# iwbn/flow-supervisor

Hardware: AMD Instinct MI355X
Metric: image-pairs/s fwd+bwd, 12 GRU iters, 436x1024 (higher is better)
Workload: dtype f32 (bf16x3 products); 1 GPU; RAFT full, 440x1024 (Sintel 436x1024 padded), 12 GRU iters, 4 pairs/GPU, train step = fwd + sequence loss + bwd + RCCL all-reduce + clip + AdamW; global_batch=4, parallelism=dp1, launch=hipGraph replay of the whole step

## Files before the change

flow_supervisor_amd/_lib.py:

```python
import ctypes
import functools
import os
from ctypes import POINTER, Structure, c_double, c_float, c_int, c_int64, c_void_p

import torch

_HERE = os.path.dirname(os.path.abspath(__file__))
LIB_PATH = os.environ.get("FSRAFT_LIB_PATH") or os.path.join(_HERE, "libfsraft.so")
_lib = None

c_float_p = c_void_p


class ConvDesc(Structure):
    _fields_ = [
        ("src", c_void_p * 3), ("srcC", c_int * 3), ("srcld", c_int * 3), ("nsrc", c_int),
        ("wpk", c_void_p), ("bias", c_void_p), ("wpk_split", c_void_p),
        ("B", c_int), ("H", c_int), ("W", c_int), ("KH", c_int), ("KW", c_int), ("N", c_int),
        ("dst", c_void_p * 3), ("dst_bs", c_int64 * 3), ("dst_ps", c_int64 * 3), ("dst_cs", c_int64 * 3),
        ("dst_n0", c_int * 3), ("dst_acc", c_int * 3), ("ndst", c_int),
        ("relu", c_int), ("alpha", c_float),
        ("epi", c_int),
        ("h", c_void_p), ("ldh", c_int), ("z", c_void_p), ("ldz", c_int),
        ("aux1", c_void_p), ("ld1", c_int), ("aux2", c_void_p), ("ld2", c_int), ("hid", c_int),
# ... 83 lines not shown
    "fsraft_inorm_relu_fwd": [c_void_p, c_void_p, c_void_p, c_int64, c_int, c_float, c_int, _S],
    "fsraft_inorm_relu_bwd": [c_void_p, c_void_p, c_void_p, c_void_p, c_int64, c_int, c_int, _S],
    "fsraft_affine_relu_fwd": [c_void_p, c_void_p, c_void_p, c_void_p, c_int64, c_int, c_int, c_int, _S],
    "fsraft_affine_relu_bwd": [c_void_p, c_void_p, c_void_p, c_void_p, c_void_p, c_void_p, c_void_p, c_int64, c_int, c_int, c_int, _S],
    "fsraft_sequence_loss": [_PP, _PP, POINTER(c_float), c_int, c_int, c_void_p, c_void_p, c_float, c_float, c_int, c_int, c_int, c_void_p, _S],
    "fsraft_corr_pool_pyramid": [_PP, c_int, c_int64, c_int, c_int, _S],
    "fsraft_corr_pool_pyramid_same": [_PP, c_int, c_int64, c_int, c_int, _S],
    "fsraft_corr_lookup_fwd_same": [_PP, c_int, c_void_p, c_int64, c_int64, c_int64, c_void_p, c_int, c_int, c_int, c_int, c_int, _S],
    "fsraft_corr_unpool_same_bwd": [_PP, c_int, c_int64, c_int, c_int, _S],
    "fsraft_corr_lookup_bwd_same": [_PP, c_int, c_void_p, c_int64, c_int64, c_int64, c_void_p, c_int, c_int, c_int, c_int, c_int, _S],
    "fsraft_corr_lookup_dcoords_same": [_PP, c_int, c_void_p, c_int64, c_int64, c_int64, c_void_p, c_int, c_void_p, c_int64, c_int64, c_int64,
                                        c_int, c_int, c_int, c_int, _S],
    "fsraft_set_norm_blocks": [c_int],
    "fsraft_get_tuning": [c_int],
    "fsraft_conv_last_route": [c_int],
    "fsraft_space_to_depth2": [c_void_p, c_void_p, c_int, c_int, c_int, c_int, c_int, _S],
    "fsraft_forward_interpolate": [c_void_p, c_void_p, c_int, c_int, _S],
    "fsraft_flow_metrics_scratch_bytes": [c_int, c_int, c_int],
    "fsraft_flow_metrics": [c_void_p, c_int64, c_int64, c_int64, c_void_p, c_int64, c_int64, c_int64, c_void_p, c_int64, c_int64,
                            c_int, c_int, c_int, c_void_p, c_void_p, c_void_p, c_int64, _S],
    "fsraft_inorm_relu_cl_fwd": [c_void_p, c_void_p, c_void_p, c_void_p, c_void_p, c_void_p, c_int, c_int, c_int, c_float, c_int, c_int, c_int, _S],
    "fsraft_inorm_relu_cl_bwd": [c_void_p, c_void_p, c_void_p, c_void_p, c_void_p, c_void_p, c_void_p, c_void_p, c_int, c_int, c_int,
                                 c_int, c_int, _S],
    "fsraft_affine_relu_cl_fwd": [c_void_p, c_void_p, c_void_p, c_void_p, c_void_p, c_int64, c_int, c_int, c_int, c_int, _S],
    "fsraft_affine_relu_cl_bwd": [c_void_p, c_void_p, c_void_p, c_void_p, c_void_p, c_void_p, c_void_p, c_void_p, c_void_p, c_int, c_int,
                                  c_int, c_int, c_int, _S],
    "fsraft_axpby": [c_void_p, c_void_p, c_float, c_float, c_int64, _S],
    "fsraft_sum_n": [_PP, c_int, c_void_p, c_int64, c_int, _S],
    "fsraft_bn_fold": [c_void_p, c_void_p, c_void_p, c_void_p, c_void_p, c_float, c_int, c_void_p, c_void_p, c_void_p, c_void_p, _S],
    "fsraft_bn_fold_bwd": [c_void_p, c_int, c_int, c_void_p, c_void_p, c_void_p, c_void_p, c_void_p, c_void_p, _S],
# ... 145 lines not shown
```

flow_supervisor_amd/csrc/conv_common.hpp:

```cpp
#pragma once
#include "gemm_core.hpp"
#include "gemm_core_split.hpp"
#include "gemm_rec.hpp"
#include <cstddef>
#include <type_traits>

struct ConvKnobs {
  int conv_tile = 0;
  int wgrad_tile = 0;
  int wgrad_blocks = 512;
  int conv_split = 1;
  int wgrad_split = 2;
  int conv_buf = 1;
  int xcd_swizzle = 0;
  int wgrad_buf = 1;
  int conv_n256 = 0;
  int wgrad_multi = 1;
  int wgrad_blocks_multi = 2048;
  int conv_uniform = 1;
  int conv_w8 = 1;
  int conv_w8_min = 64;
  int wgrad_w8 = 0;
  int wgrad_pack = 1;
  int wgrad_blocks_pack = 1024;
// ... 53 lines not shown
__device__ __forceinline__ const T* uni_ptr(const T* p) {
  const uint64_t u = reinterpret_cast<uint64_t>(p);
  return reinterpret_cast<const T*>((uint64_t)uni((unsigned)(u >> 32)) << 32 | uni((unsigned)u));
}
__device__ __forceinline__ __amdgpu_buffer_rsrc_t make_rsrc(const void* p, unsigned bytes) {
  const uint64_t u = reinterpret_cast<uint64_t>(p);
  const unsigned lo = __builtin_amdgcn_readfirstlane((unsigned)u), hi = __builtin_amdgcn_readfirstlane((unsigned)(u >> 32));
  void* q = reinterpret_cast<void*>((uint64_t)hi << 32 | lo);
  return __builtin_amdgcn_make_buffer_rsrc(q, 0, __builtin_amdgcn_readfirstlane(bytes), FS_RSRC_FLAGS);
}

using SWCfg128 = SplitTnCfg<128, 128, 2, 2, 2>;
using SWCfg128S = SplitTnCfg<128, 128, 2, 2, 1>;
using SWCfg128W8 = SplitTnCfg<128, 128, 2, 4, 1, 512>;
using SWCfgPack = SplitTnCfg<64, 192, 2, 2, 1>;
using Cfg128 = GemmCfg<128, 128, 32, 2, 2, 2, 2>;
using Cfg64 = GemmCfg<128, 64, 32, 4, 1, 2, 2>;
using CfgM64 = GemmCfg<64, 128, 32, 1, 4, 2, 2>;
using Cfg6464 = GemmCfg<64, 64, 32, 2, 2, 2, 2>;
using WCfg6464 = GemmCfg<64, 64, 32, 2, 2, 0, 0>;
using Cfg6464K16 = GemmCfg<64, 64, 16, 2, 2, 2, 2>;
using CfgM64K16 = GemmCfg<64, 128, 16, 1, 4, 2, 2>;

using SCfg128 = SplitCfg<128, 128, 2, 2>;
using SCfgN256 = SplitCfg<64, 256, 1, 4, 2, true>;
using SCfg256W16 = SplitCfg<256, 128, 4, 4, 2, true, 1024>;
using SCfg128W8 = SplitCfg<128, 128, 2, 4, 2, true, 512>;
using SCfg256N64 = SplitCfg<256, 64, 4, 2, 2, true, 512>;
using SCfgM64 = SplitCfg<64, 128, 1, 4, 2, true>;
using Cfg32 = GemmCfg<128, 32, 32, 4, 1, 2, 2>;
// ... 47 lines not shown
```

flow_supervisor_amd/csrc/conv_wgrad.hip:

```cpp
#include "conv_common.hpp"

namespace {

struct WgradArgs {
  const float* dy; int ldy; int Cout;
  Src src[3]; int nsrc;
  float* dwpk; int Ktot;
  int B, H, W, KH, KW;
  int kchunk;
  float* dbias;
  int xcd_xt, xcd_yt, xcd_groups;
};

constexpr int WGRAD_MAX_SEG = 16;
struct WgradArgsM {
  WgradArgs a;
  int nseg, zs;
  const float* dys[WGRAD_MAX_SEG];
  const float* srcs[3][WGRAD_MAX_SEG];
};

template <class Cfg>
struct ShiftedXLoader {
  static constexpr int BN = Cfg::BN, BK = Cfg::BK, LD = Cfg::LDB;
  static constexpr int F4 = BN / 4;
  static constexpr int NF4 = BK * F4 / 256;
// ... 109 lines not shown
    const int ku = __builtin_amdgcn_readfirstlane(kt);
    const unsigned w = __builtin_amdgcn_readfirstlane(mask[ku]);
    const __amdgpu_buffer_rsrc_t rs = make_rsrc(base, 0x7fffffffu);
    const unsigned soff = (unsigned)ku * 32u * ld4;
#pragma unroll
    for (int j = 0; j < NCH; ++j) {
      const unsigned voffj = voff[j] | ((__builtin_amdgcn_ubfe(w, (unsigned)krow[j], 1u) ^ 1u) << 31);
      const u32x4 v = __builtin_amdgcn_raw_buffer_load_b128(rs, voffj, soff, 0);
      const f32x4 f = __builtin_bit_cast(f32x4, v);
      r[4 * j + 0] = f[0]; r[4 * j + 1] = f[1]; r[4 * j + 2] = f[2]; r[4 * j + 3] = f[3];
    }
  }
};


template <class Cfg, bool BUF = false, bool MULTI = false>
__global__ __launch_bounds__(Cfg::NT) void conv_wgrad_split_kernel(const std::conditional_t<MULTI, WgradArgsM, WgradArgs> args) {
  static_assert(Cfg::NT == 256 || BUF, "512-thread workgroups use the buffer-addressed loaders");
  __shared__ __attribute__((aligned(16))) char lds[Cfg::LDS_BYTES];
  __shared__ unsigned pixmask[BUF ? WGRAD_MASK_WORDS : 1];
  const WgradArgs& a = [&]() -> const WgradArgs& { if constexpr (MULTI) return args.a; else return args; }();
  int bx = blockIdx.x, by = blockIdx.y, zblock = blockIdx.z, seg = 0;
  if (a.xcd_xt > 0) {
    const int span = 8 * a.xcd_xt, r = blockIdx.x / span, rem = blockIdx.x - r * span;
    const int g = r * 8 + (rem & 7);
    if (g >= a.xcd_groups) return;
    if (a.xcd_yt > 0) { bx = rem >> 3; by = g % a.xcd_yt; zblock = g / a.xcd_yt; }
    else { const int tile = rem >> 3, x0 = -a.xcd_yt; bx = tile % x0; by = tile / x0; zblock = g; }
  }
  if constexpr (MULTI) { seg = zblock / args.zs; zblock -= seg * args.zs; seg = __builtin_amdgcn_readfirstlane(seg); }
  const int HW = a.H * a.W;
  const int64_t M = (int64_t)a.B * HW;
  const int taps = a.KH * a.KW;
  int t = bx, s = 0, kofs = 0;
  for (;; ++s) {
    const int ct = (a.src[s].C + Cfg::BN - 1) / Cfg::BN;
    if (t < taps * ct) break;
    t -= taps * ct;
    kofs += taps * ((a.src[s].C + 31) / 32) * 32;
  }
  Src sc = s == 0 ? a.src[0] : s == 1 ? a.src[1] : a.src[2];
  const float* dyp = a.dy;
  if constexpr (MULTI) {
    typedef const float* fptr;
    const auto* karg = (const char __attribute__((address_space(4)))*)__builtin_amdgcn_kernarg_segment_ptr();
    dyp = ((const fptr __attribute__((address_space(4)))*)(karg + offsetof(WgradArgsM, dys)))[seg];
    sc.p = ((const fptr __attribute__((address_space(4)))*)(karg + offsetof(WgradArgsM, srcs)))[s * WGRAD_MAX_SEG + seg];
  }
  const int ct = (sc.C + Cfg::BN - 1) / Cfg::BN;
  const int tap = t / ct, ci0 = (t % ct) * Cfg::BN;
  const int cpad = ((sc.C + 31) / 32) * 32;
  kofs += tap * cpad + ci0;
  const int co0 = by * Cfg::BM;
  const int64_t mb = (int64_t)zblock * a.kchunk;
  const int64_t me = mb + a.kchunk < M ? mb + a.kchunk : M;
  if (mb >= M) return;
  const int coleft = ((a.Cout + 3) / 4) * 4 - co0;
  const int cleft = ((sc.C + 3) / 4) * 4 - ci0;
  const int dyy = tap / a.KW - a.KH / 2, dxx = tap % a.KW - a.KW / 2;
  const int KT = (int)((me - mb + 31) / 32);
  f32x16 acc[Cfg::TM][Cfg::TN];
#pragma unroll
  for (int i = 0; i < Cfg::TM; ++i)
#pragma unroll
    for (int j = 0; j < Cfg::TN; ++j)
#pragma unroll
      for (int r = 0; r < 16; ++r) acc[i][j][r] = 0.f;
  float colsum[4] = {0.f, 0.f, 0.f, 0.f};
  const bool want_bias = a.dbias != nullptr && bx == 0;
  if constexpr (BUF) {
    for (int i = threadIdx.x; i < KT * 32; i += Cfg::NT) {
      const int64_t m = mb + i;
      bool ok = m < me;
      if (ok) {
        const int pix = (int)(m % HW), yy = pix / a.W + dyy, xx = pix % a.W + dxx;
        ok = (unsigned)yy < (unsigned)a.H && (unsigned)xx < (unsigned)a.W;
      }
      const unsigned long long bal = __ballot(ok);
      if ((threadIdx.x & 63) == 0) { pixmask[i >> 5] = (unsigned)bal; pixmask[(i >> 5) + 1] = (unsigned)(bal >> 32); }
    }
    __syncthreads();
    BufDyLoader<Cfg> la;
    la.base = uni_ptr(dyp + co0 + mb * a.ldy); la.ld4 = uni((unsigned)a.ldy * 4u); la.npix = (int)(me - mb);
    const int cva = coleft < Cfg::BM ? coleft : Cfg::BM;
#pragma unroll
    for (int j = 0; j < BufDyLoader<Cfg>::NCH; ++j) {
      const int e = threadIdx.x + Cfg::NT * j, k = e / (Cfg::BM / 4), c4 = e % (Cfg::BM / 4);
      la.krow[j] = k; la.voff[j] = c4 * 4 < cva ? (unsigned)(k * a.ldy + c4 * 4) * 4u : FS_OOB;
    }
    BufShiftedXLoader<Cfg> lb;
    lb.base = uni_ptr(sc.p + ci0 + (mb + dyy * a.W + dxx) * sc.ld); lb.ld4 = uni((unsigned)sc.ld * 4u); lb.mask = pixmask;
    const int cvb = cleft < Cfg::BN ? cleft : Cfg::BN;
#pragma unroll
    for (int j = 0; j < BufShiftedXLoader<Cfg>::NCH; ++j) {
      const int e = threadIdx.x + Cfg::NT * j, k = e / (Cfg::BN / 4), c4 = e % (Cfg::BN / 4);
      lb.krow[j] = k; lb.voff[j] = c4 * 4 < cvb ? (unsigned)(k * sc.ld + c4 * 4) * 4u : FS_OOB;
    }
    if (want_bias) split_mainloop_tn<Cfg, BufDyLoader<Cfg>, BufShiftedXLoader<Cfg>, true>(lds, KT, la, lb, acc, colsum);
    else split_mainloop_tn<Cfg>(lds, KT, la, lb, acc);
  } else {
  SplitDyLoader<Cfg> la{dyp + co0, a.ldy, coleft < Cfg::BM ? coleft : Cfg::BM, mb, me};
  SplitShiftedXLoader<Cfg> lb{sc.p + ci0, sc.ld, cleft < Cfg::BN ? cleft : Cfg::BN, dyy, dxx, a.H, a.W, HW, mb, me};
  if (want_bias) split_mainloop_tn<Cfg, SplitDyLoader<Cfg>, SplitShiftedXLoader<Cfg>, true>(lds, KT, la, lb, acc, colsum);
  else split_mainloop_tn<Cfg>(lds, KT, la, lb, acc);
  }
  if (want_bias) {
    float* part = reinterpret_cast<float*>(lds);
    __syncthreads();
#pragma unroll
    for (int q = 0; q < 4; ++q) part[(threadIdx.x >> 5) * Cfg::BM + 4 * (threadIdx.x & 31) + q] = colsum[q];
    __syncthreads();
    if (threadIdx.x < Cfg::BM) {
      float s = 0.f;
#pragma unroll
      for (int g = 0; g < Cfg::NT / 32; ++g) s += part[g * Cfg::BM + threadIdx.x];
      if (co0 + threadIdx.x < a.Cout) atomicAdd(a.dbias + co0 + threadIdx.x, s);
    }
  }
#pragma unroll
  for (int nt = 0; nt < Cfg::TN; ++nt) {
    const int n = acc_col<Cfg>(nt);
    if (ci0 + n >= cpad) continue;
#pragma unroll
    for (int mt = 0; mt < Cfg::TM; ++mt)
#pragma unroll
      for (int r = 0; r < 16; ++r) {
        const int co = co0 + acc_row<Cfg>(mt, r);
        if (co < a.Cout) atomicAdd(a.dwpk + (int64_t)co * a.Ktot + kofs + n, acc[mt][nt][r]);
      }
  }
}

constexpr int WGRAD_PACK_WORDS = 256;
constexpr int WGRAD_PACK_SLOTS = 8;

template <class Cfg>
struct BufPackedXLoader {
  static constexpr int NCH = Cfg::NCH_B, NREG = NCH * 4;
  const float* base; unsigned ld4; const unsigned* mask;
  unsigned voff[NCH]; int krow[NCH]; int slot[NCH];
  __device__ __forceinline__ void fetch_tile(int kt, float (&r)[NREG]) const {
    const int ku = __builtin_amdgcn_readfirstlane(kt);
    const __amdgpu_buffer_rsrc_t rs = make_rsrc(base, 0x7fffffffu);
// ... 156 lines not shown
    if (ci0 + n >= cpad) continue;
#pragma unroll
    for (int mt = 0; mt < Cfg::TM; ++mt)
#pragma unroll
      for (int r = 0; r < 16; ++r) {
        const int co = co0 + acc_row<Cfg>(mt, r);
        if (co < a.Cout) atomicAdd(a.dwpk + (int64_t)co * a.Ktot + kofs + n, acc[mt][nt][r]);
      }
  }
}

}

#include "wgrad_patch.inc"

extern "C" int fsraft_conv_wgrad(const float* dy, int ldy, int Cout, const float* const* src, const int* srcC,
                                 const int* srcld, int nsrc, float* dwpk, float* dbias, int B, int H, int W, int KH,
                                 int KW, hipStream_t stream) {
  if (!dy || !src || !dwpk || nsrc < 1 || nsrc > 3 || ldy % 4 != 0) return FS_ERR_ARG;
  t_route[1] = 0;
  WgradArgs a{};
  a.dy = dy; a.ldy = ldy; a.Cout = Cout;
  const bool small_m = Cout <= 32;
  const bool t64 = !small_m && knob.wgrad_tile == 3;
  const int bn = t64 ? 64 : 128, bm = small_m ? 32 : (t64 ? 64 : 128);
  if (!fill_srcs(a.src, src, srcC, srcld, nsrc)) return FS_ERR_ARG;
  int xt128 = 0;
  for (int s = 0; s < nsrc; ++s) xt128 += KH * KW * ceil_div(srcC[s], bn);
  a.nsrc = nsrc; a.dwpk = dwpk; a.Ktot = conv_ktot(srcC, nsrc, KH * KW);
  a.B = B; a.H = H; a.W = W; a.KH = KH; a.KW = KW;
  const int64_t M = (int64_t)B * H * W;
  if (knob.wgrad_patch && knob.wgrad_patch1 && knob.wgrad_split != 0 && KH == 3 && KW == 3 && Cout > 32 && M >= knob.wgrad_patch1) {
    WgradArgsM m{};
    m.a = a; m.a.dbias = dbias;
    m.nseg = 1;
// ... 4 lines not shown
  }
  if (knob.wgrad_pack && knob.wgrad_split != 0 && knob.wgrad_buf && nsrc == 1 && srcC[0] <= 96 && KH * KW > 1 &&
      (int64_t)(32 * (WGRAD_PACK_WORDS - 2) + 2 * W + 2) * srcld[0] * 4 < 0x7fffffff) {
    const int cpad = ceil_div(srcC[0], 32) * 32;
    int tp = SWCfgPack::BN / cpad;
    if (tp > WGRAD_PACK_SLOTS) tp = WGRAD_PACK_SLOTS;
    const int xt = ceil_div(KH * KW, tp), yt = ceil_div(Cout, SWCfgPack::BM);
    const int64_t chunk = wgrad_chunk(knob.wgrad_blocks_pack, (int64_t)xt * yt, M, WGRAD_PACK_WORDS);
    a.kchunk = (int)chunk;
    a.dbias = dbias;
    dim3 grid(xt, yt, (unsigned)((M + chunk - 1) / chunk));
    if (knob.wgrad_xcd == 2) {
      a.xcd_xt = xt; a.xcd_yt = yt; a.xcd_groups = yt * (int)grid.z;
      grid = dim3((unsigned)(ceil_div(a.xcd_groups, 8) * 8 * xt), 1, 1);
    }
    t_route[1] = 6;
    hipLaunchKernelGGL((conv_wgrad_pack_kernel<SWCfgPack>), grid, dim3(SWCfgPack::NT), 0, stream, a);
    return fs_launch_status();
  }
  const int ytiles = ceil_div(Cout, bm);
  const int64_t chunk = wgrad_chunk(knob.wgrad_blocks, (int64_t)xt128 * ytiles, M, WGRAD_MASK_WORDS);
  a.kchunk = (int)chunk;
  const int zs = (int)((M + chunk - 1) / chunk);
  dim3 grid(xt128, ytiles, zs);
  a.dbias = dbias;
  const bool wbuf = knob.wgrad_buf && chunk <= 32 * (WGRAD_MASK_WORDS - 2) && (int64_t)chunk * 4 * 2048 < 0x7fffffff;
  if (!small_m && !t64 && knob.wgrad_split == 1) {
    t_route[1] = 4;
    if (wbuf) hipLaunchKernelGGL((conv_wgrad_split_kernel<SWCfg128, true>), grid, dim3(256), 0, stream, a);
    else hipLaunchKernelGGL((conv_wgrad_split_kernel<SWCfg128>), grid, dim3(256), 0, stream, a);
    return fs_launch_status();
  }
  if (!small_m && !t64 && knob.wgrad_split == 2) {
    t_route[1] = 5;
    if (wbuf) hipLaunchKernelGGL((conv_wgrad_split_kernel<SWCfg128S, true>), grid, dim3(256), 0, stream, a);
    else hipLaunchKernelGGL((conv_wgrad_split_kernel<SWCfg128S>), grid, dim3(256), 0, stream, a);
    return fs_launch_status();
  }
  if (dbias) { const int rc = fsraft_col_sum(dy, ldy, M, Cout, dbias, 1.0f, stream); if (rc) return rc; }
  t_route[1] = small_m ? 1 : t64 ? 2 : 3;
  if (small_m) hipLaunchKernelGGL((conv_wgrad_kernel<WCfg32>), grid, dim3(256), 0, stream, a);
  else if (t64) hipLaunchKernelGGL((conv_wgrad_kernel<WCfg6464>), grid, dim3(256), 0, stream, a);
  else hipLaunchKernelGGL((conv_wgrad_kernel<WCfg128>), grid, dim3(256), 0, stream, a);
  return fs_launch_status();
}

extern "C" int fsraft_conv_wgrad_multi(const float* const* dy, int nseg, int ldy, int Cout, const float* const* src,
                                       const int* srcC, const int* srcld, int nsrc, float* dwpk, float* dbias, int B,
                                       int H, int W, int KH, int KW, hipStream_t stream) {
  if (!dy || !src || !dwpk || nseg < 1 || nsrc < 1 || nsrc > 3 || ldy % 4 != 0) return FS_ERR_ARG;
  t_route[1] = 0;
  const int64_t M = (int64_t)B * H * W;
  const bool fast = knob.wgrad_multi && nseg > 1 && Cout > 32 && knob.wgrad_tile != 3 && knob.wgrad_split == 2 && knob.wgrad_buf;
  for (int base = 0; base < nseg; base += WGRAD_MAX_SEG) {
    const int n = nseg - base < WGRAD_MAX_SEG ? nseg - base : WGRAD_MAX_SEG;
    if (!fast || n == 1) {
      for (int i = 0; i < n; ++i) {
        const int rc = fsraft_conv_wgrad(dy[base + i], ldy, Cout, src + (size_t)(base + i) * nsrc, srcC, srcld, nsrc, dwpk,
                                         dbias, B, H, W, KH, KW, stream);
        if (rc) return rc;
      }
      continue;
    }
    WgradArgsM m{};
    WgradArgs& a = m.a;
    a.dy = dy[base]; a.ldy = ldy; a.Cout = Cout;
// ... 7 lines not shown
        if (!src[(size_t)(base + i) * nsrc + s]) return FS_ERR_ARG;
        m.srcs[s][i] = src[(size_t)(base + i) * nsrc + s];
      }
    }
    a.nsrc = nsrc; a.dwpk = dwpk; a.Ktot = conv_ktot(srcC, nsrc, KH * KW);
    a.B = B; a.H = H; a.W = W; a.KH = KH; a.KW = KW; a.dbias = dbias;
    if (knob.wgrad_patch && KH * KW > 1) {
      m.nseg = n;
      const int rc = launch_wgrad_patch(m, stream);
      if (rc == 0) continue;
      if (rc > 0) return rc;
    }
    const int ytiles = ceil_div(Cout, 128);
    const int64_t chunk = wgrad_chunk(knob.wgrad_blocks_multi, (int64_t)xt128 * ytiles * n, M, WGRAD_MASK_WORDS);
    if ((int64_t)chunk * 4 * 2048 >= 0x7fffffff) return FS_ERR_ARG;
    a.kchunk = (int)chunk;
    m.zs = (int)((M + chunk - 1) / chunk);
    m.nseg = n;
    dim3 grid(xt128, ytiles, m.zs * n);
    if (knob.wgrad_xcd == 3) {
      m.a.xcd_xt = xt128 * ytiles; m.a.xcd_yt = -xt128; m.a.xcd_groups = m.zs * n;
      grid = dim3((unsigned)(ceil_div(m.a.xcd_groups, 8) * 8 * xt128 * ytiles), 1, 1);
    } else if (knob.wgrad_xcd) {
      m.a.xcd_xt = xt128; m.a.xcd_yt = ytiles; m.a.xcd_groups = ytiles * m.zs * n;
      grid = dim3((unsigned)(ceil_div(m.a.xcd_groups, 8) * 8 * xt128), 1, 1);
    }
    t_route[1] = knob.wgrad_w8 ? 9 : 8;
    if (knob.wgrad_w8) hipLaunchKernelGGL((conv_wgrad_split_kernel<SWCfg128W8, true, true>), grid, dim3(512), 0, stream, m);
    else hipLaunchKernelGGL((conv_wgrad_split_kernel<SWCfg128S, true, true>), grid, dim3(256), 0, stream, m);
    const int rc = fs_launch_status();
// ... 5 lines not shown
```

flow_supervisor_amd/csrc/gemm_core_split.hpp:

```cpp
#pragma once
#include "common.hpp"
#include <type_traits>

typedef __bf16 bf16x8 __attribute__((ext_vector_type(8)));
typedef __bf16 bf16x4 __attribute__((ext_vector_type(4)));

template <class L, class = void>
struct has_fetch_tile : std::false_type {};
template <class L>
struct has_fetch_tile<L, std::void_t<decltype(&L::fetch_tile)>> : std::true_type {};
template <class L, int N>
__device__ __forceinline__ void fetch_all(const L& l, int kt, float (&r)[N]) {
  if constexpr (has_fetch_tile<L>::value) {
    l.fetch_tile(kt, r);
  } else {
#pragma unroll
    for (int c = 0; c < L::NCH; ++c) l.fetch_chunk(kt, r, c);
  }
}

template <int BM_, int BN_, int WM_, int WN_, int NBUF_ = 2, bool SWZ_ = false, int NT_ = 256>
struct SplitCfg {
  static constexpr int NT = NT_;
  static constexpr int NBUF = NBUF_;
  static constexpr int BM = BM_, BN = BN_, BK = 32, WM = WM_, WN = WN_;
// ... 184 lines not shown
  uint2 hi, lo;
  split4(r, hi, lo);
  char* p = tile + (e / (COLS / 4)) * PITCH + (e % (COLS / 4)) * 8;
  *reinterpret_cast<uint2*>(p) = hi;
  *reinterpret_cast<uint2*>(p + PLANE) = lo;
}

__device__ __forceinline__ bf16x8 tr_frag(const char* p, int pitch) {
  const s16x4 a = __builtin_amdgcn_ds_read_tr16_b64_v4i16((s16x4 __attribute__((address_space(3)))*)(p));
  const s16x4 b = __builtin_amdgcn_ds_read_tr16_b64_v4i16((s16x4 __attribute__((address_space(3)))*)(p + 4 * pitch));
  typedef short s16x8 __attribute__((ext_vector_type(8)));
  const s16x8 v = {a[0], a[1], a[2], a[3], b[0], b[1], b[2], b[3]};
  return __builtin_bit_cast(bf16x8, v);
}

template <class Cfg, class LA, class LB, bool COLSUM = false>
__device__ __forceinline__ void split_mainloop_tn(char* __restrict__ lds, int KT, const LA& la, const LB& lb,
                                                  f32x16 (&acc)[Cfg::TM][Cfg::TN], float* colsum = nullptr) {
  static_assert(LA::NCH == Cfg::NCH_A && LB::NCH == Cfg::NCH_B, "loader tile shape must match the config");
  const int lane = threadIdx.x & 63, wave = threadIdx.x >> 6;
  const int wm = wave / Cfg::WN, wn = wave % Cfg::WN;
  const int lh = lane >> 5, gb = (lane >> 4) & 1, q = (lane & 15) >> 2, p4 = lane & 3;

  float ra[LA::NREG], rb[LB::NREG];
  auto stage = [&](char* dst, bool count) {
#pragma unroll
    for (int c = 0; c < LA::NCH; ++c) {
      stage_convert_kmajor<Cfg::BM, Cfg::PA, Cfg::A_PLANE>(dst, threadIdx.x + Cfg::NT * c, ra + 4 * c);
      if (COLSUM && count) {
#pragma unroll
        for (int q = 0; q < 4; ++q) colsum[q] += ra[4 * c + q];
      }
    }
#pragma unroll
    for (int c = 0; c < LB::NCH; ++c)
      stage_convert_kmajor<Cfg::BN, Cfg::PB, Cfg::B_PLANE>(dst + 2 * Cfg::A_PLANE, threadIdx.x + Cfg::NT * c, rb + 4 * c);
  };
  if (KT > 0) {
    fetch_all(la, 0, ra);
    fetch_all(lb, 0, rb);
    stage(lds, true);
  }
  __syncthreads();
  for (int kt = 0; kt < KT; ++kt) {
    char* cur = lds + (Cfg::NBUF == 2 ? (kt & 1) * Cfg::STAGE : 0);
    char* nxt = lds + (Cfg::NBUF == 2 ? ((kt + 1) & 1) * Cfg::STAGE : 0);
    const int ktn = (kt + 1 < KT) ? kt + 1 : kt;
    fetch_all(la, ktn, ra);
    fetch_all(lb, ktn, rb);
    const char* As = cur + (8 * lh + q) * Cfg::PA + (wm * (Cfg::TM * 32) + 16 * gb + 4 * p4) * 2;
    const char* Bs = cur + 2 * Cfg::A_PLANE + (8 * lh + q) * Cfg::PB + (wn * (Cfg::TN * 32) + 16 * gb + 4 * p4) * 2;
#pragma unroll
    for (int s = 0; s < 2; ++s) {
      bf16x8 ah[Cfg::TM], al[Cfg::TM], bh[Cfg::TN], bl[Cfg::TN];
#pragma unroll
      for (int mt = 0; mt < Cfg::TM; ++mt) {
        ah[mt] = tr_frag(As + s * 16 * Cfg::PA + mt * 64, Cfg::PA);
        al[mt] = tr_frag(As + s * 16 * Cfg::PA + mt * 64 + Cfg::A_PLANE, Cfg::PA);
      }
#pragma unroll
      for (int nt = 0; nt < Cfg::TN; ++nt) {
        bh[nt] = tr_frag(Bs + s * 16 * Cfg::PB + nt * 64, Cfg::PB);
        bl[nt] = tr_frag(Bs + s * 16 * Cfg::PB + nt * 64 + Cfg::B_PLANE, Cfg::PB);
      }
#pragma unroll
      for (int mt = 0; mt < Cfg::TM; ++mt)
#pragma unroll
        for (int nt = 0; nt < Cfg::TN; ++nt) {
          acc[mt][nt] = __builtin_amdgcn_mfma_f32_32x32x16_bf16(al[mt], bh[nt], acc[mt][nt], 0, 0, 0);
          acc[mt][nt] = __builtin_amdgcn_mfma_f32_32x32x16_bf16(ah[mt], bl[nt], acc[mt][nt], 0, 0, 0);
          acc[mt][nt] = __builtin_amdgcn_mfma_f32_32x32x16_bf16(ah[mt], bh[nt], acc[mt][nt], 0, 0, 0);
        }
    }
    if (Cfg::NBUF == 1) __syncthreads();
    stage(nxt, kt + 1 < KT);
    __syncthreads();
  }
}
```

include/fsraft_tuning.h:

```cpp
#ifndef FSRAFT_TUNING_H
#define FSRAFT_TUNING_H

#ifdef __cplusplus
extern "C" {
#endif

enum fsraft_tuning_key {
  FSRAFT_KEY_CONV_TILE = 0,
  FSRAFT_KEY_WGRAD_TILE = 1,
  FSRAFT_KEY_WGRAD_BLOCKS = 2,
  FSRAFT_KEY_CONV_ARITH = 3,
  FSRAFT_KEY_WGRAD_ARITH = 4,
  FSRAFT_KEY_CONV_BUF = 5,
  FSRAFT_KEY_XCD_SWIZZLE = 7,
  FSRAFT_KEY_WGRAD_BUF = 8,
  FSRAFT_KEY_CONV_N256 = 9,
  FSRAFT_KEY_WGRAD_MULTI = 10,
  FSRAFT_KEY_WGRAD_BLOCKS_MULTI = 11,
  FSRAFT_KEY_CONV_UNIFORM = 12,
  FSRAFT_KEY_CONV_W8 = 13,
  FSRAFT_KEY_CONV_W8_MIN = 14,
  FSRAFT_KEY_WGRAD_W8 = 15,
  FSRAFT_KEY_WGRAD_PACK = 16,
  FSRAFT_KEY_WGRAD_BLOCKS_PACK = 17,
  FSRAFT_KEY_CONV_N64 = 18,
  FSRAFT_KEY_CONV_N64_MIN_M = 19,
  FSRAFT_KEY_CONV_HALO = 20,
  FSRAFT_KEY_CONV_HALO_MIN_M = 21,
  FSRAFT_KEY_WGRAD_XCD = 22,
  FSRAFT_KEY_CONV_PATCH = 26,
  FSRAFT_KEY_WGRAD_PATCH = 27,
  FSRAFT_KEY_CONV_PATCH64 = 28,
  FSRAFT_KEY_WGRAD_PATCH1 = 29,
  FSRAFT_KEY_CONV_PATCH_MIN_M = 31,
  FSRAFT_KEY_CONV_KSPLIT = 32
};
int fsraft_set_tuning(int key, int value);
int fsraft_get_tuning(int key);
int fsraft_conv_last_route(int which);
int fsraft_set_build_split(int on);
int fsraft_set_build_kernel(int which);
int fsraft_set_lookup_policy(int aux);
int fsraft_set_ktile_exact(int levels);
int fsraft_set_upsample_kernel(int v4);
int fsraft_set_dvol_box(int on);
int fsraft_set_dvol_policy(int policy);
int fsraft_set_gemm_split(int on);
int fsraft_set_lookup_qb(int qb);
int fsraft_set_norm_blocks(int target_workgroups);
int fsraft_set_rec_mfma16(int on);
int fsraft_set_alt_tile(int on);

#ifdef __cplusplus
}
// ... 3 lines not shown
```

Measured before the change: 114.4 image-pairs/s.

## Add wide 256-column wgrad tiles with warp-specialized pipelined mainloop

Adds a wide weight-gradient path that pairs two 128-channel input groups into one 256-column tile, with 256 or 128 output rows and 512-thread workgroups. Each half of the workgroup builds its own pixel mask and loads its own x half, and leftover row and column tiles go to the existing 128x128 kernel. The split mainloop gains a PIPE mode in which half the waves stage the next tile before computing and the other half after, to overlap LDS staging with MFMA work. The aim is more data reuse per tile and fewer atomic partial-sum launches, at the cost of higher register and LDS pressure, extra launches for the remainder tiles, and a more complex chunk plan.

```diff
diff --git a/flow_supervisor_amd/_lib.py b/flow_supervisor_amd/_lib.py
--- a/flow_supervisor_amd/_lib.py
+++ b/flow_supervisor_amd/_lib.py
@@ -121,6 +121,8 @@
     "fsraft_set_norm_blocks": [c_int],
     "fsraft_get_tuning": [c_int],
     "fsraft_conv_last_route": [c_int],
+    "fsraft_set_wgrad_wide": [c_int],
+    "fsraft_conv_wgrad_last_tile": [],
     "fsraft_space_to_depth2": [c_void_p, c_void_p, c_int, c_int, c_int, c_int, c_int, _S],
     "fsraft_forward_interpolate": [c_void_p, c_void_p, c_int, c_int, _S],
     "fsraft_flow_metrics_scratch_bytes": [c_int, c_int, c_int],
diff --git a/flow_supervisor_amd/csrc/conv_common.hpp b/flow_supervisor_amd/csrc/conv_common.hpp
--- a/flow_supervisor_amd/csrc/conv_common.hpp
+++ b/flow_supervisor_amd/csrc/conv_common.hpp
@@ -91,6 +91,8 @@
 using SWCfg128S = SplitTnCfg<128, 128, 2, 2, 1>;
 using SWCfg128W8 = SplitTnCfg<128, 128, 2, 4, 1, 512>;
 using SWCfgPack = SplitTnCfg<64, 192, 2, 2, 1>;
+using SWCfgW256 = SplitTnCfg<256, 256, 2, 4, 2, 512>;
+using SWCfgW128 = SplitTnCfg<128, 256, 2, 4, 2, 512>;
 using Cfg128 = GemmCfg<128, 128, 32, 2, 2, 2, 2>;
 using Cfg64 = GemmCfg<128, 64, 32, 4, 1, 2, 2>;
 using CfgM64 = GemmCfg<64, 128, 32, 1, 4, 2, 2>;
diff --git a/flow_supervisor_amd/csrc/conv_wgrad.hip b/flow_supervisor_amd/csrc/conv_wgrad.hip
--- a/flow_supervisor_amd/csrc/conv_wgrad.hip
+++ b/flow_supervisor_amd/csrc/conv_wgrad.hip
@@ -10,6 +10,7 @@
   int kchunk;
   float* dbias;
   int xcd_xt, xcd_yt, xcd_groups;
+  int bx0, by0;
 };
 
 constexpr int WGRAD_MAX_SEG = 16;
@@ -149,11 +150,37 @@
 };
 
 
+constexpr int WGRAD_WIDE_WORDS = 512;
+template <class Cfg>
+struct BufWideXLoader : BufShiftedXLoader<Cfg> {
+  int e0;
+  __device__ __forceinline__ int elem(int c) const { return e0 + 8 * (Cfg::BN / 4) * c; }
+};
+
+struct XGroup { int s, tap, ci0, kofs, cpad; };
+template <int GW>
+__device__ __forceinline__ XGroup wgrad_xgroup(const WgradArgs& a, int t, int taps) {
+  int s = 0, kofs = 0;
+  for (;; ++s) {
+    const int ct = (a.src[s].C + GW - 1) / GW;
+    if (t < taps * ct) break;
+    t -= taps * ct;
+    kofs += taps * ((a.src[s].C + 31) / 32) * 32;
+  }
+  const int C = s == 0 ? a.src[0].C : s == 1 ? a.src[1].C : a.src[2].C;
+  const int ct = (C + GW - 1) / GW, cpad = ((C + 31) / 32) * 32;
+  const int tap = t / ct, ci0 = (t % ct) * GW;
+  return XGroup{s, tap, ci0, kofs + tap * cpad + ci0, cpad};
+}
+
 template <class Cfg, bool BUF = false, bool MULTI = false>
 __global__ __launch_bounds__(Cfg::NT) void conv_wgrad_split_kernel(const std::conditional_t<MULTI, WgradArgsM, WgradArgs> args) {
   static_assert(Cfg::NT == 256 || BUF, "512-thread workgroups use the buffer-addressed loaders");
+  constexpr bool WIDE = Cfg::BN == 256;
+  static_assert(!WIDE || (BUF && Cfg::NT == 512), "the 256-column x tile is loaded by two halves of 256 threads");
+  constexpr int GW = WIDE ? 128 : Cfg::BN;
   __shared__ __attribute__((aligned(16))) char lds[Cfg::LDS_BYTES];
-  __shared__ unsigned pixmask[BUF ? WGRAD_MASK_WORDS : 1];
+  __shared__ unsigned pixmask[BUF ? (WIDE ? 2 * WGRAD_WIDE_WORDS : WGRAD_MASK_WORDS) : 1];
   const WgradArgs& a = [&]() -> const WgradArgs& { if constexpr (MULTI) return args.a; else return args; }();
   int bx = blockIdx.x, by = blockIdx.y, zblock = blockIdx.z, seg = 0;
   if (a.xcd_xt > 0) {
@@ -164,16 +191,15 @@
     else { const int tile = rem >> 3, x0 = -a.xcd_yt; bx = tile % x0; by = tile / x0; zblock = g; }
   }
   if constexpr (MULTI) { seg = zblock / args.zs; zblock -= seg * args.zs; seg = __builtin_amdgcn_readfirstlane(seg); }
+  bx += a.bx0; by += a.by0;
   const int HW = a.H * a.W;
   const int64_t M = (int64_t)a.B * HW;
   const int taps = a.KH * a.KW;
-  int t = bx, s = 0, kofs = 0;
-  for (;; ++s) {
-    const int ct = (a.src[s].C + Cfg::BN - 1) / Cfg::BN;
-    if (t < taps * ct) break;
-    t -= taps * ct;
-    kofs += taps * ((a.src[s].C + 31) / 32) * 32;
-  }
+  const int wave = __builtin_amdgcn_readfirstlane((int)(threadIdx.x >> 6));
+  const int xh = WIDE ? wave >> 2 : 0, oh = WIDE ? ((wave % Cfg::WN) * (Cfg::TN * 32)) >> 7 : 0;
+  const XGroup gl = wgrad_xgroup<GW>(a, WIDE ? 2 * bx + xh : bx, taps);
+  const XGroup go = WIDE ? wgrad_xgroup<GW>(a, 2 * bx + oh, taps) : gl;
+  const int s = gl.s;
   Src sc = s == 0 ? a.src[0] : s == 1 ? a.src[1] : a.src[2];
   const float* dyp = a.dy;
   if constexpr (MULTI) {
@@ -182,10 +208,7 @@
     dyp = ((const fptr __attribute__((address_space(4)))*)(karg + offsetof(WgradArgsM, dys)))[seg];
     sc.p = ((const fptr __attribute__((address_space(4)))*)(karg + offsetof(WgradArgsM, srcs)))[s * WGRAD_MAX_SEG + seg];
   }
-  const int ct = (sc.C + Cfg::BN - 1) / Cfg::BN;
-  const int tap = t / ct, ci0 = (t % ct) * Cfg::BN;
-  const int cpad = ((sc.C + 31) / 32) * 32;
-  kofs += tap * cpad + ci0;
+  const int tap = gl.tap, ci0 = gl.ci0;
   const int co0 = by * Cfg::BM;
   const int64_t mb = (int64_t)zblock * a.kchunk;
   const int64_t me = mb + a.kchunk < M ? mb + a.kchunk : M;
@@ -204,7 +227,9 @@
   float colsum[4] = {0.f, 0.f, 0.f, 0.f};
   const bool want_bias = a.dbias != nullptr && bx == 0;
   if constexpr (BUF) {
-    for (int i = threadIdx.x; i < KT * 32; i += Cfg::NT) {
+    constexpr int MT = WIDE ? 256 : Cfg::NT;
+    unsigned* pm = pixmask + xh * WGRAD_WIDE_WORDS;
+    for (int i = threadIdx.x % MT; i < KT * 32; i += MT) {
       const int64_t m = mb + i;
       bool ok = m < me;
       if (ok) {
@@ -212,7 +237,7 @@
         ok = (unsigned)yy < (unsigned)a.H && (unsigned)xx < (unsigned)a.W;
       }
       const unsigned long long bal = __ballot(ok);
-      if ((threadIdx.x & 63) == 0) { pixmask[i >> 5] = (unsigned)bal; pixmask[(i >> 5) + 1] = (unsigned)(bal >> 32); }
+      if ((threadIdx.x & 63) == 0) { pm[i >> 5] = (unsigned)bal; pm[(i >> 5) + 1] = (unsigned)(bal >> 32); }
     }
     __syncthreads();
     BufDyLoader<Cfg> la;
@@ -223,16 +248,26 @@
       const int e = threadIdx.x + Cfg::NT * j, k = e / (Cfg::BM / 4), c4 = e % (Cfg::BM / 4);
       la.krow[j] = k; la.voff[j] = c4 * 4 < cva ? (unsigned)(k * a.ldy + c4 * 4) * 4u : FS_OOB;
     }
-    BufShiftedXLoader<Cfg> lb;
-    lb.base = uni_ptr(sc.p + ci0 + (mb + dyy * a.W + dxx) * sc.ld); lb.ld4 = uni((unsigned)sc.ld * 4u); lb.mask = pixmask;
-    const int cvb = cleft < Cfg::BN ? cleft : Cfg::BN;
-#pragma unroll
-    for (int j = 0; j < BufShiftedXLoader<Cfg>::NCH; ++j) {
-      const int e = threadIdx.x + Cfg::NT * j, k = e / (Cfg::BN / 4), c4 = e % (Cfg::BN / 4);
-      lb.krow[j] = k; lb.voff[j] = c4 * 4 < cvb ? (unsigned)(k * sc.ld + c4 * 4) * 4u : FS_OOB;
-    }
-    if (want_bias) split_mainloop_tn<Cfg, BufDyLoader<Cfg>, BufShiftedXLoader<Cfg>, true>(lds, KT, la, lb, acc, colsum);
-    else split_mainloop_tn<Cfg>(lds, KT, la, lb, acc);
+    std::conditional_t<WIDE, BufWideXLoader<Cfg>, BufShiftedXLoader<Cfg>> lb;
+    lb.base = uni_ptr(sc.p + ci0 + (mb + dyy * a.W + dxx) * sc.ld); lb.ld4 = uni((unsigned)sc.ld * 4u); lb.mask = pm;
+    const int cvb = cleft < GW ? cleft : GW;
+    if constexpr (WIDE) {
+      const int t8 = threadIdx.x & 255, c4 = t8 & 31;
+#pragma unroll
+      for (int j = 0; j < BufShiftedXLoader<Cfg>::NCH; ++j) {
+        const int k = (t8 >> 5) + 8 * j;
+        lb.krow[j] = k; lb.voff[j] = c4 * 4 < cvb ? (unsigned)(k * sc.ld + c4 * 4) * 4u : FS_OOB;
+      }
+      lb.e0 = (t8 >> 5) * (Cfg::BN / 4) + xh * 32 + c4;
+    } else {
+#pragma unroll
+      for (int j = 0; j < BufShiftedXLoader<Cfg>::NCH; ++j) {
+        const int e = threadIdx.x + Cfg::NT * j, k = e / (Cfg::BN / 4), c4 = e % (Cfg::BN / 4);
+        lb.krow[j] = k; lb.voff[j] = c4 * 4 < cvb ? (unsigned)(k * sc.ld + c4 * 4) * 4u : FS_OOB;
+      }
+    }
+    if (want_bias) split_mainloop_tn<Cfg, BufDyLoader<Cfg>, decltype(lb), true, WIDE>(lds, KT, la, lb, acc, colsum);
+    else split_mainloop_tn<Cfg, BufDyLoader<Cfg>, decltype(lb), false, WIDE>(lds, KT, la, lb, acc);
   } else {
   SplitDyLoader<Cfg> la{dyp + co0, a.ldy, coleft < Cfg::BM ? coleft : Cfg::BM, mb, me};
   SplitShiftedXLoader<Cfg> lb{sc.p + ci0, sc.ld, cleft < Cfg::BN ? cleft : Cfg::BN, dyy, dxx, a.H, a.W, HW, mb, me};
@@ -240,28 +275,29 @@
   else split_mainloop_tn<Cfg>(lds, KT, la, lb, acc);
   }
   if (want_bias) {
+    constexpr int Q = Cfg::BM / 4, G = Cfg::NT / Q;
     float* part = reinterpret_cast<float*>(lds);
     __syncthreads();
 #pragma unroll
-    for (int q = 0; q < 4; ++q) part[(threadIdx.x >> 5) * Cfg::BM + 4 * (threadIdx.x & 31) + q] = colsum[q];
+    for (int q = 0; q < 4; ++q) part[(threadIdx.x / Q) * Cfg::BM + 4 * (threadIdx.x % Q) + q] = colsum[q];
     __syncthreads();
     if (threadIdx.x < Cfg::BM) {
       float s = 0.f;
 #pragma unroll
-      for (int g = 0; g < Cfg::NT / 32; ++g) s += part[g * Cfg::BM + threadIdx.x];
+      for (int g = 0; g < G; ++g) s += part[g * Cfg::BM + threadIdx.x];
       if (co0 + threadIdx.x < a.Cout) atomicAdd(a.dbias + co0 + threadIdx.x, s);
     }
   }
 #pragma unroll
   for (int nt = 0; nt < Cfg::TN; ++nt) {
-    const int n = acc_col<Cfg>(nt);
-    if (ci0 + n >= cpad) continue;
+    const int n = acc_col<Cfg>(nt) & (GW - 1);
+    if (go.ci0 + n >= go.cpad) continue;
 #pragma unroll
     for (int mt = 0; mt < Cfg::TM; ++mt)
 #pragma unroll
       for (int r = 0; r < 16; ++r) {
         const int co = co0 + acc_row<Cfg>(mt, r);
-        if (co < a.Cout) atomicAdd(a.dwpk + (int64_t)co * a.Ktot + kofs + n, acc[mt][nt][r]);
+        if (co < a.Cout) atomicAdd(a.dwpk + (int64_t)co * a.Ktot + go.kofs + n, acc[mt][nt][r]);
       }
   }
 }
@@ -448,11 +484,86 @@
 
 #include "wgrad_patch.inc"
 
+namespace {
+int g_wgrad_wide = 1;
+__thread int t_wgrad_tile = 0;
+
+struct WidePlan {
+  int bm;
+  int pairs, groups;
+  int yw;
+  int64_t chunk;
+};
+
+WidePlan wide_plan(int Cout, const int* srcC, int nsrc, int taps, int64_t M, int nseg, int64_t chunk128) {
+  WidePlan p{};
+  if (g_wgrad_wide == 0 || Cout <= 32) return p;
+  for (int s = 0; s < nsrc; ++s) p.groups += taps * ceil_div(srcC[s], 128);
+  p.pairs = p.groups / 2;
+  if (p.pairs == 0) return p;
+  const int bm = Cout >= 256 ? 256 : 128;
+  const int yw = bm == 256 ? Cout / 256 : ceil_div(Cout, 128);
+  const int64_t tiles = (int64_t)p.pairs * yw * nseg, s128 = (M + chunk128 - 1) / chunk128;
+  int64_t want = 512 / tiles;
+  if (want > s128) want = s128;
+  if (tiles * want > 256) want = 256 * (tiles * want / 256) / tiles;
+  if (want < 1) want = 1;
+  int64_t chunk = (M + want - 1) / want;
+  if (chunk < 256) chunk = 256;
+  chunk = (chunk + 31) / 32 * 32;
+  if (chunk > 32 * (WGRAD_WIDE_WORDS - 2) || chunk * 4 * 2048 >= 0x7fffffff) return p;
+  if (g_wgrad_wide == 1) {
+    if (tiles * ((M + chunk - 1) / chunk) < 192 || chunk < 512) return p;
+  }
+  p.bm = bm; p.yw = yw; p.chunk = chunk;
+  return p;
+}
+
+template <class Cfg, bool MULTI, class A>
+int launch_split(A m, int xt, int yt, int zs, int nseg, int bx0, int by0, int64_t chunk, int xcd, hipStream_t stream) {
+  WgradArgs& a = [&]() -> WgradArgs& { if constexpr (MULTI) return m.a; else return m; }();
+  a.kchunk = (int)chunk; a.bx0 = bx0; a.by0 = by0;
+  a.xcd_xt = a.xcd_yt = a.xcd_groups = 0;
+  if constexpr (MULTI) { m.zs = zs; m.nseg = nseg; }
+  dim3 grid(xt, yt, zs * nseg);
+  if (xcd == 3) {
+    a.xcd_xt = xt * yt; a.xcd_yt = -xt; a.xcd_groups = zs * nseg;
+    grid = dim3((unsigned)(ceil_div(a.xcd_groups, 8) * 8 * xt * yt), 1, 1);
+  } else if (xcd) {
+    a.xcd_xt = xt; a.xcd_yt = yt; a.xcd_groups = yt * zs * nseg;
+    grid = dim3((unsigned)(ceil_div(a.xcd_groups, 8) * 8 * xt), 1, 1);
+  }
+  hipLaunchKernelGGL((conv_wgrad_split_kernel<Cfg, true, MULTI>), grid, dim3(Cfg::NT), 0, stream, m);
+  return fs_launch_status();
+}
+
+template <bool MULTI, class A>
+int launch_wide(const A& m, const WidePlan& p, int Cout, int64_t M, int nseg, int64_t chunk128, int xcd, hipStream_t stream) {
+  const int zsw = (int)((M + p.chunk - 1) / p.chunk), zs = (int)((M + chunk128 - 1) / chunk128);
+  int rc = p.bm == 256 ? launch_split<SWCfgW256, MULTI>(m, p.pairs, p.yw, zsw, nseg, 0, 0, p.chunk, xcd, stream)
+                       : launch_split<SWCfgW128, MULTI>(m, p.pairs, p.yw, zsw, nseg, 0, 0, p.chunk, xcd, stream);
+  if (rc) return rc;
+  const int y128 = ceil_div(Cout, 128), ydone = p.bm == 256 ? 2 * p.yw : p.yw;
+  if (ydone < y128) rc = launch_split<SWCfg128S, MULTI>(m, p.groups, y128 - ydone, zs, nseg, 0, ydone, chunk128, xcd, stream);
+  if (rc) return rc;
+  if (p.groups & 1) rc = launch_split<SWCfg128S, MULTI>(m, 1, ydone, zs, nseg, p.groups - 1, 0, chunk128, xcd, stream);
+  t_wgrad_tile = p.bm << 16 | 256;
+  return rc;
+}
+}
+
+extern "C" int fsraft_set_wgrad_wide(int mode) {
+  if (mode < 0 || mode > 2) return FS_ERR_ARG;
+  g_wgrad_wide = mode;
+  return FS_OK;
+}
+extern "C" int fsraft_conv_wgrad_last_tile(void) { return t_wgrad_tile; }
+
 extern "C" int fsraft_conv_wgrad(const float* dy, int ldy, int Cout, const float* const* src, const int* srcC,
                                  const int* srcld, int nsrc, float* dwpk, float* dbias, int B, int H, int W, int KH,
                                  int KW, hipStream_t stream) {
   if (!dy || !src || !dwpk || nsrc < 1 || nsrc > 3 || ldy % 4 != 0) return FS_ERR_ARG;
-  t_route[1] = 0;
+  t_route[1] = 0; t_wgrad_tile = 0;
   WgradArgs a{};
   a.dy = dy; a.ldy = ldy; a.Cout = Cout;
   const bool small_m = Cout <= 32;
@@ -487,7 +598,7 @@
       a.xcd_xt = xt; a.xcd_yt = yt; a.xcd_groups = yt * (int)grid.z;
       grid = dim3((unsigned)(ceil_div(a.xcd_groups, 8) * 8 * xt), 1, 1);
     }
-    t_route[1] = 6;
+    t_route[1] = 6; t_wgrad_tile = SWCfgPack::BM << 16 | SWCfgPack::BN;
     hipLaunchKernelGGL((conv_wgrad_pack_kernel<SWCfgPack>), grid, dim3(SWCfgPack::NT), 0, stream, a);
     return fs_launch_status();
   }
@@ -499,19 +610,25 @@
   a.dbias = dbias;
   const bool wbuf = knob.wgrad_buf && chunk <= 32 * (WGRAD_MASK_WORDS - 2) && (int64_t)chunk * 4 * 2048 < 0x7fffffff;
   if (!small_m && !t64 && knob.wgrad_split == 1) {
-    t_route[1] = 4;
+    t_route[1] = 4; t_wgrad_tile = 128 << 16 | 128;
     if (wbuf) hipLaunchKernelGGL((conv_wgrad_split_kernel<SWCfg128, true>), grid, dim3(256), 0, stream, a);
     else hipLaunchKernelGGL((conv_wgrad_split_kernel<SWCfg128>), grid, dim3(256), 0, stream, a);
     return fs_launch_status();
   }
   if (!small_m && !t64 && knob.wgrad_split == 2) {
     t_route[1] = 5;
-    if (wbuf) hipLaunchKernelGGL((conv_wgrad_split_kernel<SWCfg128S, true>), grid, dim3(256), 0, stream, a);
+    t_wgrad_tile = 128 << 16 | 128;
+    if (wbuf) {
+      const WidePlan p = wide_plan(Cout, srcC, nsrc, KH * KW, M, 1, chunk);
+      if (p.bm) return launch_wide<false>(a, p, Cout, M, 1, chunk, 0, stream);
+    }
+    if (wbuf)hipLaunchKernelGGL((conv_wgrad_split_kernel<SWCfg128S, true>), grid, dim3(256), 0, stream, a);
     else hipLaunchKernelGGL((conv_wgrad_split_kernel<SWCfg128S>), grid, dim3(256), 0, stream, a);
     return fs_launch_status();
   }
   if (dbias) { const int rc = fsraft_col_sum(dy, ldy, M, Cout, dbias, 1.0f, stream); if (rc) return rc; }
   t_route[1] = small_m ? 1 : t64 ? 2 : 3;
+  t_wgrad_tile = bm << 16 | bn;
   if (small_m) hipLaunchKernelGGL((conv_wgrad_kernel<WCfg32>), grid, dim3(256), 0, stream, a);
   else if (t64) hipLaunchKernelGGL((conv_wgrad_kernel<WCfg6464>), grid, dim3(256), 0, stream, a);
   else hipLaunchKernelGGL((conv_wgrad_kernel<WCfg128>), grid, dim3(256), 0, stream, a);
@@ -522,7 +639,7 @@
                                        const int* srcC, const int* srcld, int nsrc, float* dwpk, float* dbias, int B,
                                        int H, int W, int KH, int KW, hipStream_t stream) {
   if (!dy || !src || !dwpk || nseg < 1 || nsrc < 1 || nsrc > 3 || ldy % 4 != 0) return FS_ERR_ARG;
-  t_route[1] = 0;
+  t_route[1] = 0; t_wgrad_tile = 0;
   const int64_t M = (int64_t)B * H * W;
   const bool fast = knob.wgrad_multi && nseg > 1 && Cout > 32 && knob.wgrad_tile != 3 && knob.wgrad_split == 2 && knob.wgrad_buf;
   for (int base = 0; base < nseg; base += WGRAD_MAX_SEG) {
@@ -560,6 +677,16 @@
     const int ytiles = ceil_div(Cout, 128);
     const int64_t chunk = wgrad_chunk(knob.wgrad_blocks_multi, (int64_t)xt128 * ytiles * n, M, WGRAD_MASK_WORDS);
     if ((int64_t)chunk * 4 * 2048 >= 0x7fffffff) return FS_ERR_ARG;
+    if (!knob.wgrad_w8) {
+      const WidePlan p = wide_plan(Cout, srcC, nsrc, KH * KW, M, n, chunk);
+      if (p.bm) {
+        t_route[1] = 8;
+        const int rc = launch_wide<true>(m, p, Cout, M, n, chunk, knob.wgrad_xcd, stream);
+        if (rc) return rc;
+        continue;
+      }
+    }
+    t_wgrad_tile = 128 << 16 | 128;
     a.kchunk = (int)chunk;
     m.zs = (int)((M + chunk - 1) / chunk);
     m.nseg = n;
diff --git a/flow_supervisor_amd/csrc/gemm_core_split.hpp b/flow_supervisor_amd/csrc/gemm_core_split.hpp
--- a/flow_supervisor_amd/csrc/gemm_core_split.hpp
+++ b/flow_supervisor_amd/csrc/gemm_core_split.hpp
@@ -9,6 +9,15 @@
 struct has_fetch_tile : std::false_type {};
 template <class L>
 struct has_fetch_tile<L, std::void_t<decltype(&L::fetch_tile)>> : std::true_type {};
+template <class L, class = void>
+struct has_elem : std::false_type {};
+template <class L>
+struct has_elem<L, std::void_t<decltype(&L::elem)>> : std::true_type {};
+template <int NT, class L>
+__device__ __forceinline__ int chunk_elem(const L& l, int c) {
+  if constexpr (has_elem<L>::value) return l.elem(c);
+  else return threadIdx.x + NT * c;
+}
 template <class L, int N>
 __device__ __forceinline__ void fetch_all(const L& l, int kt, float (&r)[N]) {
   if constexpr (has_fetch_tile<L>::value) {
@@ -223,7 +232,7 @@
   return __builtin_bit_cast(bf16x8, v);
 }
 
-template <class Cfg, class LA, class LB, bool COLSUM = false>
+template <class Cfg, class LA, class LB, bool COLSUM = false, bool PIPE = false>
 __device__ __forceinline__ void split_mainloop_tn(char* __restrict__ lds, int KT, const LA& la, const LB& lb,
                                                   f32x16 (&acc)[Cfg::TM][Cfg::TN], float* colsum = nullptr) {
   static_assert(LA::NCH == Cfg::NCH_A && LB::NCH == Cfg::NCH_B, "loader tile shape must match the config");
@@ -243,12 +252,70 @@
     }
 #pragma unroll
     for (int c = 0; c < LB::NCH; ++c)
-      stage_convert_kmajor<Cfg::BN, Cfg::PB, Cfg::B_PLANE>(dst + 2 * Cfg::A_PLANE, threadIdx.x + Cfg::NT * c, rb + 4 * c);
+      stage_convert_kmajor<Cfg::BN, Cfg::PB, Cfg::B_PLANE>(dst + 2 * Cfg::A_PLANE, chunk_elem<Cfg::NT>(lb, c), rb + 4 * c);
+  };
+  auto compute = [&](const char* cur) {
+    const char* As = cur + (8 * lh + q) * Cfg::PA + (wm * (Cfg::TM * 32) + 16 * gb + 4 * p4) * 2;
+    const char* Bs = cur + 2 * Cfg::A_PLANE + (8 * lh + q) * Cfg::PB + (wn * (Cfg::TN * 32) + 16 * gb + 4 * p4) * 2;
+#pragma unroll
+    for (int s = 0; s < 2; ++s) {
+      bf16x8 ah[Cfg::TM], al[Cfg::TM], bh[Cfg::TN], bl[Cfg::TN];
+#pragma unroll
+      for (int mt = 0; mt < Cfg::TM; ++mt) {
+        ah[mt] = tr_frag(As + s * 16 * Cfg::PA + mt * 64, Cfg::PA);
+        al[mt] = tr_frag(As + s * 16 * Cfg::PA + mt * 64 + Cfg::A_PLANE, Cfg::PA);
+      }
+#pragma unroll
+      for (int nt = 0; nt < Cfg::TN; ++nt) {
+        bh[nt] = tr_frag(Bs + s * 16 * Cfg::PB + nt * 64, Cfg::PB);
+        bl[nt] = tr_frag(Bs + s * 16 * Cfg::PB + nt * 64 + Cfg::B_PLANE, Cfg::PB);
+      }
+#pragma unroll
+      for (int mt = 0; mt < Cfg::TM; ++mt)
+#pragma unroll
+        for (int nt = 0; nt < Cfg::TN; ++nt) {
+          acc[mt][nt] = __builtin_amdgcn_mfma_f32_32x32x16_bf16(al[mt], bh[nt], acc[mt][nt], 0, 0, 0);
+          acc[mt][nt] = __builtin_amdgcn_mfma_f32_32x32x16_bf16(ah[mt], bl[nt], acc[mt][nt], 0, 0, 0);
+          acc[mt][nt] = __builtin_amdgcn_mfma_f32_32x32x16_bf16(ah[mt], bh[nt], acc[mt][nt], 0, 0, 0);
+        }
+    }
   };
   if (KT > 0) {
     fetch_all(la, 0, ra);
     fetch_all(lb, 0, rb);
     stage(lds, true);
+  }
+  if constexpr (PIPE) {
+    static_assert(Cfg::NBUF == 2, "staging tile kt + 1 while tile kt is read needs two LDS images");
+    if (KT > 1) {
+      fetch_all(la, 1, ra);
+      fetch_all(lb, 1, rb);
+    }
+    __syncthreads();
+    auto advance = [&](int kt) {
+      if (kt + 1 < KT) {
+        stage(lds + ((kt + 1) & 1) * Cfg::STAGE, true);
+        const int k2 = kt + 2 < KT ? kt + 2 : KT - 1;
+        fetch_all(la, k2, ra);
+        fetch_all(lb, k2, rb);
+      }
+    };
+    if (__builtin_amdgcn_readfirstlane(wave) < Cfg::NT / 128) {
+      for (int kt = 0; kt < KT; ++kt) {
+        advance(kt);
+        __builtin_amdgcn_sched_barrier(0);
+        compute(lds + (kt & 1) * Cfg::STAGE);
+        __syncthreads();
+      }
+    } else {
+      for (int kt = 0; kt < KT; ++kt) {
+        compute(lds + (kt & 1) * Cfg::STAGE);
+        __builtin_amdgcn_sched_barrier(0);
+        advance(kt);
+        __syncthreads();
+      }
+    }
+    return;
   }
   __syncthreads();
   for (int kt = 0; kt < KT; ++kt) {
@@ -257,30 +324,7 @@
     const int ktn = (kt + 1 < KT) ? kt + 1 : kt;
     fetch_all(la, ktn, ra);
     fetch_all(lb, ktn, rb);
-    const char* As = cur + (8 * lh + q) * Cfg::PA + (wm * (Cfg::TM * 32) + 16 * gb + 4 * p4) * 2;
-    const char* Bs = cur + 2 * Cfg::A_PLANE + (8 * lh + q) * Cfg::PB + (wn * (Cfg::TN * 32) + 16 * gb + 4 * p4) * 2;
-#pragma unroll
-    for (int s = 0; s < 2; ++s) {
-      bf16x8 ah[Cfg::TM], al[Cfg::TM], bh[Cfg::TN], bl[Cfg::TN];
-#pragma unroll
-      for (int mt = 0; mt < Cfg::TM; ++mt) {
-        ah[mt] = tr_frag(As + s * 16 * Cfg::PA + mt * 64, Cfg::PA);
-        al[mt] = tr_frag(As + s * 16 * Cfg::PA + mt * 64 + Cfg::A_PLANE, Cfg::PA);
-      }
-#pragma unroll
-      for (int nt = 0; nt < Cfg::TN; ++nt) {
-        bh[nt] = tr_frag(Bs + s * 16 * Cfg::PB + nt * 64, Cfg::PB);
-        bl[nt] = tr_frag(Bs + s * 16 * Cfg::PB + nt * 64 + Cfg::B_PLANE, Cfg::PB);
-      }
-#pragma unroll
-      for (int mt = 0; mt < Cfg::TM; ++mt)
-#pragma unroll
-        for (int nt = 0; nt < Cfg::TN; ++nt) {
-          acc[mt][nt] = __builtin_amdgcn_mfma_f32_32x32x16_bf16(al[mt], bh[nt], acc[mt][nt], 0, 0, 0);
-          acc[mt][nt] = __builtin_amdgcn_mfma_f32_32x32x16_bf16(ah[mt], bl[nt], acc[mt][nt], 0, 0, 0);
-          acc[mt][nt] = __builtin_amdgcn_mfma_f32_32x32x16_bf16(ah[mt], bh[nt], acc[mt][nt], 0, 0, 0);
-        }
-    }
+    compute(cur);
     if (Cfg::NBUF == 1) __syncthreads();
     stage(nxt, kt + 1 < KT);
     __syncthreads();
diff --git a/include/fsraft_tuning.h b/include/fsraft_tuning.h
--- a/include/fsraft_tuning.h
+++ b/include/fsraft_tuning.h
@@ -38,6 +38,8 @@
 int fsraft_set_tuning(int key, int value);
 int fsraft_get_tuning(int key);
 int fsraft_conv_last_route(int which);
+int fsraft_set_wgrad_wide(int mode);
+int fsraft_conv_wgrad_last_tile(void);
 int fsraft_set_build_split(int on);
 int fsraft_set_build_kernel(int which);
 int fsraft_set_lookup_policy(int aux);
```

Result: faster. 115.6 image-pairs/s (median of 6 runs) (+1.0%).
